# sharinka0715/semantic-gaussians

Measured on NVIDIA H100. Metric: Mviews/s + HBM GB/s, 1M Gaussians, 256-ch features, 1080p, fwd+bwd, higher is better.
Workload: dtype f32

## Files before the change

### semantic-gaussians_b200/csrc/blend_bwd.cu

```cuda
#include <cstdlib>
#include "common.cuh"

namespace sgb {

namespace {

constexpr int kThreads = SGB_TILE_PIX;
constexpr int kWarps = kThreads / 32;
constexpr int kBatchB = 32;
constexpr int CH = 4;

struct __align__(16) BwdSmem {
    float4 recA[2][kBatchB];
    float4 recB[2][kBatchB];
    uint32_t ids[2][kBatchB];
    float feat[2][kBatchB][CH];
    float dF[kWarps][kBatchB][CH];
    float geo[kWarps][kBatchB][8];
    uint32_t active[kWarps];
};

__device__ __forceinline__ float warp_sum(float v) {
#pragma unroll
    for (int o = 16; o >= 1; o >>= 1) v += __shfl_xor_sync(0xffffffffu, v, o);
    return v;
}

__global__ void __launch_bounds__(kThreads) blend_backward_kernel(
    const uint2* __restrict__ ranges, const uint32_t* __restrict__ point_list, int W, int H, int C,
    const float* __restrict__ bg_color, const SplatRec* __restrict__ rec, const float* __restrict__ colors,
    const float* __restrict__ final_Ts, const uint32_t* __restrict__ n_contrib,
    const uint32_t* __restrict__ tile_last, const float* __restrict__ dL_dpixels, float* __restrict__ dL_dmean2D,
    float* __restrict__ dL_dconic2D, float* __restrict__ dL_dopacity, float* __restrict__ dL_dcolors) {
    extern __shared__ __align__(128) unsigned char smem_raw[];
    BwdSmem& sm = *reinterpret_cast<BwdSmem*>(smem_raw);

    const int tiles_x = (W + SGB_TILE - 1) / SGB_TILE;
    const int tile = blockIdx.x;
    const int ch0 = blockIdx.y * CH;
    const int nch = min(CH, C - ch0);
    const int tid = threadIdx.x, lane = tid & 31, warp = tid >> 5;
    const uint32_t tx = tid & (SGB_TILE - 1), ty = tid >> 4;
    const uint2 pix = {(uint32_t)(tile % tiles_x) * SGB_TILE + tx, (uint32_t)(tile / tiles_x) * SGB_TILE + ty};
    const uint32_t pix_id = W * pix.y + pix.x;
    const float2 pixf = {(float)pix.x, (float)pix.y};
    const bool inside = pix.x < (uint32_t)W && pix.y < (uint32_t)H;
    const uint2 range = ranges[tile];
    const int total = (int)min(tile_last[tile], range.y - range.x);
    const int nbatches = (total + kBatchB - 1) / kBatchB;
    if (nbatches == 0) return;

    if (nch < CH)
        for (int e = tid; e < 2 * kBatchB * CH; e += kThreads) {
            const int k = e % CH;
            if (k >= nch) (&sm.feat[0][0][0])[e] = 0.f;
        }
    __syncthreads();

    auto issue = [&](int b) {
        const int st = b & 1;
        const int hi = total - b * kBatchB;
        const int cnt = min(kBatchB, hi);
        if (tid < cnt) {
            const uint32_t id = point_list[range.x + hi - 1 - tid];
            sm.ids[st][tid] = id;
            const float4* rp = reinterpret_cast<const float4*>(rec + id);
            sm.recA[st][tid] = __ldg(rp);
            sm.recB[st][tid] = __ldg(rp + 1);
        }
        for (int e = tid; e < cnt * nch; e += kThreads) {
            const int j = e / nch, k = e - j * nch;
            const uint32_t id = point_list[range.x + hi - 1 - j];
            sm.feat[st][j][k] = __ldg(colors + (size_t)id * C + ch0 + k);
        }
    };

    float dL[CH];
    float bgdot = 0.f;
    const size_t plane = (size_t)H * W;
#pragma unroll
    for (int k = 0; k < CH; k++) {
        dL[k] = (inside && k < nch) ? __ldg(dL_dpixels + (size_t)(ch0 + k) * plane + pix_id) : 0.f;
        if (k < nch) bgdot += bg_color[ch0 + k] * dL[k];
    }
    const float T_final = inside ? final_Ts[pix_id] : 0.f;
    float T = T_final;
    const int last_contributor = inside ? (int)n_contrib[pix_id] : 0;
    float last_alpha = 0.f, s_last = 0.f, A = 0.f;
    const float ddelx_dx = 0.5f * W, ddely_dy = 0.5f * H;

    issue(0);
    for (int b = 0; b < nbatches; b++) {
        const int st = b & 1;
        const int hi = total - b * kBatchB;
        const int cnt = min(kBatchB, hi);
        __syncthreads();
        if (b + 1 < nbatches) issue(b + 1);
        __syncthreads();
        uint32_t my_active = 0;

        for (int j = 0; j < cnt; j++) {
            const int pos = hi - 1 - j;
            const float4 a = sm.recA[st][j];
            const float4 con_o = sm.recB[st][j];
            const float2 d = {a.x - pixf.x, a.y - pixf.y};
            const float power = -0.5f * (con_o.x * d.x * d.x + con_o.z * d.y * d.y) - con_o.y * d.x * d.y;
            const float G = exp(power);
            const float alpha = min(0.99f, con_o.w * G);
            const bool contributes = (pos < last_contributor) && !(power > 0.0f) && !(alpha < 1.0f / 255.0f);
            if (!__any_sync(0xffffffffu, contributes)) continue;

            float w = 0.f, g0 = 0.f, g1 = 0.f, g2 = 0.f, g3 = 0.f, g4 = 0.f, g5 = 0.f;
            if (contributes) {
                T = T / (1.f - alpha);
                w = alpha * T;
                float s = 0.f;
#pragma unroll
                for (int k = 0; k < CH; k++) s += sm.feat[st][j][k] * dL[k];
                A = last_alpha * s_last + (1.f - last_alpha) * A;
                s_last = s;
                float dL_dalpha = (s - A) * T;
                last_alpha = alpha;
                dL_dalpha += (-T_final / (1.f - alpha)) * bgdot;
                const float dL_dG = con_o.w * dL_dalpha;
                const float gdx = G * d.x, gdy = G * d.y;
                const float dG_ddelx = -gdx * con_o.x - gdy * con_o.y;
                const float dG_ddely = -gdy * con_o.z - gdx * con_o.y;
                g0 = dL_dG * dG_ddelx * ddelx_dx;
                g1 = dL_dG * dG_ddely * ddely_dy;
                g2 = -0.5f * gdx * d.x * dL_dG;
                g3 = -0.5f * gdx * d.y * dL_dG;
                g4 = -0.5f * gdy * d.y * dL_dG;
                g5 = G * dL_dalpha;
            }
            g0 = warp_sum(g0); g1 = warp_sum(g1); g2 = warp_sum(g2);
            g3 = warp_sum(g3); g4 = warp_sum(g4); g5 = warp_sum(g5);
            if (lane == 0) {
                float* gp = sm.geo[warp][j];
                *reinterpret_cast<float4*>(gp) = make_float4(g0, g1, g2, g3);
                *reinterpret_cast<float2*>(gp + 4) = make_float2(g4, g5);
            }
#pragma unroll
            for (int k = 0; k < CH; k++) {
                const float t = warp_sum(w * dL[k]);
                if (lane == 0) sm.dF[warp][j][k] = t;
            }
            my_active |= 1u << j;
        }
        if (lane == 0) sm.active[warp] = my_active;
        __syncthreads();

        for (int e = tid; e < cnt * CH; e += kThreads) {
            const int j = e / CH, k = e - j * CH;
            if (k >= nch) continue;
            float t = 0.f;
            bool any = false;
#pragma unroll
            for (int wv = 0; wv < kWarps; wv++)
                if (sm.active[wv] >> j & 1u) { t += sm.dF[wv][j][k]; any = true; }
            if (any) red_add_f32(dL_dcolors + (size_t)sm.ids[st][j] * C + ch0 + k, t);
        }
        for (int e = tid; e < cnt * 6; e += kThreads) {
            const int j = e / 6, q = e - j * 6;
            float t = 0.f;
            bool any = false;
#pragma unroll
            for (int wv = 0; wv < kWarps; wv++)
                if (sm.active[wv] >> j & 1u) { t += sm.geo[wv][j][q]; any = true; }
            if (any) {
                const size_t id = sm.ids[st][j];
                float* dst = q < 2 ? dL_dmean2D + id * 3 + q
                           : q < 5 ? dL_dconic2D + id * 4 + (q == 4 ? 3 : q - 2)
                                   : dL_dopacity + id;
                red_add_f32(dst, t);
            }
        }
    }
}

}

int launch_blend_backward(const sgb_view_inputs& in, GeomView g, BinView b, ImgView im, const float* colors,
                          const float* dL_dpix, float* dL_dmean2D, float* dL_dconic, float* dL_dopacity,
                          float* dL_dcolors, cudaStream_t s) {
    if (in.C > 4) {
        set_error("launch_blend_backward handles C <= 4 only");
        return SGB_E_INVALID;
    }
    const int tiles = ((in.W + SGB_TILE - 1) / SGB_TILE) * ((in.H + SGB_TILE - 1) / SGB_TILE);
    const int chunks = (in.C + CH - 1) / CH;
    const size_t smem = sizeof(BwdSmem);
    static DeviceOnce attr_set;
    if (attr_set.first_use_on_device()) {
        SGB_CUDA(cudaFuncSetAttribute(blend_backward_kernel, cudaFuncAttributeMaxDynamicSharedMemorySize, (int)smem));
    }
    blend_backward_kernel<<<dim3(tiles, chunks), kThreads, smem, s>>>(
        im.ranges, b.point_list, in.W, in.H, in.C, in.background, g.rec, colors, im.final_T, im.n_contrib,
        im.tile_last, dL_dpix, dL_dmean2D, dL_dconic, dL_dopacity, dL_dcolors);
    SGB_LAUNCH_CHECK("blend_backward_kernel", in.debug, s);
    return SGB_OK;
}

}
```

### semantic-gaussians_b200/csrc/blend_fwd.cu

```cuda
#include <cstdlib>
#include "common.cuh"

namespace sgb {

namespace {

constexpr int kThreads = SGB_TILE_PIX;
constexpr int kBatch = 64;
constexpr int CH = 4;

struct __align__(16) FwdStage {
    float4 recA[kBatch];
    float4 recB[kBatch];
    float feat[kBatch][CH];
};

template <bool DEPTH>
__global__ void __launch_bounds__(kThreads) blend_forward_kernel(
    const uint2* __restrict__ ranges, const uint32_t* __restrict__ point_list, int W, int H, int C,
    const SplatRec* __restrict__ rec, const float* __restrict__ features, const float* __restrict__ bg_color,
    float* __restrict__ final_T, uint32_t* __restrict__ n_contrib, uint32_t* __restrict__ tile_last,
    float* __restrict__ out_color, float* __restrict__ out_depth) {
    extern __shared__ __align__(128) unsigned char smem_raw[];
    FwdStage* stage = reinterpret_cast<FwdStage*>(smem_raw);
    __shared__ uint32_t s_last;

    const int tiles_x = (W + SGB_TILE - 1) / SGB_TILE;
    const int tile = blockIdx.x;
    const int ch0 = blockIdx.y * CH;
    const int nch = min(CH, C - ch0);
    const int tid = threadIdx.x;
    const uint32_t tx = tid & (SGB_TILE - 1), ty = tid >> 4;
    const uint2 pix_min = {(uint32_t)(tile % tiles_x) * SGB_TILE, (uint32_t)(tile / tiles_x) * SGB_TILE};
    const uint2 pix = {pix_min.x + tx, pix_min.y + ty};
    const uint32_t pix_id = W * pix.y + pix.x;
    const float2 pixf = {(float)pix.x, (float)pix.y};
    const bool inside = pix.x < (uint32_t)W && pix.y < (uint32_t)H;
    bool done = !inside;

    const uint2 range = ranges[tile];
    const int total = (int)(range.y - range.x);
    const int nbatches = (total + kBatch - 1) / kBatch;

    if (tid == 0) s_last = 0;
    __syncthreads();

    auto issue = [&](int b) {
        FwdStage& st = stage[b & 1];
        const int base = b * kBatch;
        const int cnt = min(kBatch, total - base);
        if (tid < cnt) {
            const uint32_t id = point_list[range.x + base + tid];
            const float4* rp = reinterpret_cast<const float4*>(rec + id);
            st.recA[tid] = __ldg(rp);
            st.recB[tid] = __ldg(rp + 1);
        }
        for (int e = tid; e < cnt * nch; e += kThreads) {
            const int j = e / nch, k = e - j * nch;
            const uint32_t id = point_list[range.x + base + j];
            st.feat[j][k] = __ldg(features + (size_t)id * C + ch0 + k);
        }
    };

    float T = 1.0f;
    uint32_t contributor = 0;
    uint32_t last_contributor = 0;
    float D = 15.0f;
    float acc[CH];
#pragma unroll
    for (int k = 0; k < CH; k++) acc[k] = 0.f;

    if (nbatches > 0) issue(0);

    for (int b = 0; b < nbatches; b++) {
        const int num_done = __syncthreads_count(done);
        if (num_done == kThreads) break;
        if (b + 1 < nbatches) issue(b + 1);
        __syncthreads();

        const FwdStage& st = stage[b & 1];
        const int cnt = min(kBatch, total - b * kBatch);
        for (int j = 0; !done && j < cnt; j++) {
            contributor++;
            const float4 a = st.recA[j];
            const float2 xy = {a.x, a.y};
            const float2 d = {xy.x - pixf.x, xy.y - pixf.y};
            const float4 con_o = st.recB[j];
            const float power = -0.5f * (con_o.x * d.x * d.x + con_o.z * d.y * d.y) - con_o.y * d.x * d.y;
            if (power > 0.0f) continue;
            const float alpha = min(0.99f, con_o.w * exp(power));
            if (alpha < 1.0f / 255.0f) continue;
            const float test_T = T * (1 - alpha);
            if (test_T < 0.0001f) {
                done = true;
                continue;
            }
#pragma unroll
            for (int k = 0; k < CH; k++)
                if (k < nch) acc[k] += st.feat[j][k] * alpha * T;
            if (DEPTH) {
                if (T > 0.5f && test_T < 0.5) D = a.z;
            }
            T = test_T;
            last_contributor = contributor;
        }
    }

    if (blockIdx.y == 0) {
        if (inside) {
            final_T[pix_id] = T;
            n_contrib[pix_id] = last_contributor;
            if (DEPTH) out_depth[pix_id] = D;
            atomicMax(&s_last, last_contributor);
        }
        __syncthreads();
        if (tid == 0) tile_last[tile] = s_last;
    }
    if (inside) {
        const size_t plane = (size_t)H * W;
#pragma unroll
        for (int k = 0; k < CH; k++)
            if (k < nch) out_color[(size_t)(ch0 + k) * plane + pix_id] = acc[k] + T * bg_color[ch0 + k];
    }
}

template <bool DEPTH>
int launch_one(const sgb_view_inputs& in, GeomView g, BinView b, ImgView im, const float* colors,
               float* out_color, float* out_depth, cudaStream_t s) {
    const int tiles = ((in.W + SGB_TILE - 1) / SGB_TILE) * ((in.H + SGB_TILE - 1) / SGB_TILE);
    const int chunks = (in.C + CH - 1) / CH;
    const size_t smem = 2 * sizeof(FwdStage);
    auto kern = blend_forward_kernel<DEPTH>;
    static DeviceOnce attr_set;
    if (attr_set.first_use_on_device()) {
        SGB_CUDA(cudaFuncSetAttribute(kern, cudaFuncAttributeMaxDynamicSharedMemorySize, (int)smem));
    }
    kern<<<dim3(tiles, chunks), kThreads, smem, s>>>(im.ranges, b.point_list, in.W, in.H, in.C, g.rec, colors,
                                                    in.background, im.final_T, im.n_contrib, im.tile_last,
                                                    out_color, out_depth);
    SGB_LAUNCH_CHECK("blend_forward_kernel", in.debug, s);
    return SGB_OK;
}

}

int launch_blend_forward(const sgb_view_inputs& in, GeomView g, BinView b, ImgView im, const float* colors,
                         float* out_color, float* out_depth, cudaStream_t s) {
    if (in.C > 4) {
        set_error("launch_blend_forward handles C <= 4 only");
        return SGB_E_INVALID;
    }
    if (out_depth) return launch_one<true>(in, g, b, im, colors, out_color, out_depth, s);
    return launch_one<false>(in, g, b, im, colors, out_color, nullptr, s);
}

}
```

### semantic-gaussians_b200/csrc/blend_v3.cu

```cuda
#include <cstddef>
#include <cstring>
#include <cuda.h>
#include "common.cuh"
#include "blend_pool.cuh"

namespace sgb {

namespace {

constexpr int kThreads = SGB_TILE_PIX;

__device__ __forceinline__ int lane_group8(int lane) { return (lane & 1) | (((lane >> 2) & 3) << 1); }
__device__ __forceinline__ int lane_group4(int lane) { return ((lane >> 1) & 1) | ((lane >> 4) << 1); }

constexpr int kAB = 32;

struct __align__(16) AlphaSmem {
    float4 recA[kAB];
    float4 recB[kAB];
    uint32_t ids[kAB];
    float wbuf[kAB][SGB_TILE_PIX];
    uint32_t wmask[8];
    uint32_t slot_chunk[kAB];
    uint32_t cur_chunk;
    uint32_t s_last;
};

__global__ void __launch_bounds__(kThreads) alpha_pass_kernel(
    const uint2* __restrict__ ranges, const uint32_t* __restrict__ point_list, int W, int H,
    const SplatRec* __restrict__ rec, float* __restrict__ final_T, uint32_t* __restrict__ n_contrib,
    uint32_t* __restrict__ tile_last, PoolView pool) {
    extern __shared__ __align__(128) unsigned char smem_raw[];
    AlphaSmem& sm = *reinterpret_cast<AlphaSmem*>(smem_raw);

    const int tiles_x = (W + SGB_TILE - 1) / SGB_TILE;
    const int tile = blockIdx.x;
    const int tid = threadIdx.x, lane = tid & 31, warp = tid >> 5;
    const uint32_t tx = tid & (SGB_TILE - 1), ty = tid >> 4;
    const uint2 pix = {(uint32_t)(tile % tiles_x) * SGB_TILE + tx, (uint32_t)(tile / tiles_x) * SGB_TILE + ty};
    const uint32_t pix_id = W * pix.y + pix.x;
    const float2 pixf = {(float)pix.x, (float)pix.y};
    const bool inside = pix.x < (uint32_t)W && pix.y < (uint32_t)H;
    bool done = !inside;

    const uint2 range = ranges[tile];
    const int total = (int)(range.y - range.x);
    const int nbatches = (total + kAB - 1) / kAB;
    const uint32_t dbase = range.x / kChunkEntries + (uint32_t)tile;
    if (tid == 0) { sm.cur_chunk = kNone; sm.s_last = 0; }

    float T = 1.0f;
    uint32_t last_contributor = 0;
    uint32_t n_tile = 0;
    uint32_t n_blend = 0;

    auto load_id = [&](int bb) -> uint32_t {
        const int i = bb * kAB + tid;
        return (tid < kAB && bb < nbatches && i < total) ? __ldg(point_list + range.x + i) : 0u;
    };
    uint32_t id_cur = load_id(0), id_nxt = load_id(1);
    float4 rA = make_float4(0.f, 0.f, 0.f, 0.f), rB = rA;
    if (tid < kAB && tid < total) {
        const float4* rp = reinterpret_cast<const float4*>(rec + id_cur);
        rA = __ldg(rp);
        rB = __ldg(rp + 1);
    }
    for (int b = 0; b < nbatches; b++) {
        const int num_done = __syncthreads_count(done);
        if (num_done == kThreads) break;
        const int base = b * kAB;
        const int cnt = min(kAB, total - base);
        if (tid < cnt) {
            sm.ids[tid] = id_cur;
            sm.recA[tid] = rA;
            sm.recB[tid] = rB;
        }
        __syncthreads();
        if (tid < kAB) {
            id_cur = id_nxt;
            if (base + kAB + tid < total) {
                const float4* rp = reinterpret_cast<const float4*>(rec + id_cur);
                rA = __ldg(rp);
                rB = __ldg(rp + 1);
            }
            id_nxt = load_id(b + 2);
        }
        uint32_t my_mask = 0;
        for (int j = 0; j < cnt; j++) {
            float w = 0.f;
            if (!done) {
                const float4 a = sm.recA[j];
                const float2 xy = {a.x, a.y};
                const float2 d = {xy.x - pixf.x, xy.y - pixf.y};
                const float4 con_o = sm.recB[j];
                const float power = -0.5f * (con_o.x * d.x * d.x + con_o.z * d.y * d.y) - con_o.y * d.x * d.y;
                if (!(power > 0.0f)) {
                    const float alpha = min(0.99f, con_o.w * exp(power));
                    if (!(alpha < 1.0f / 255.0f)) {
                        const float test_T = T * (1 - alpha);
                        if (test_T < 0.0001f) {
                            done = true;
                        } else {
                            w = alpha * T;
                            T = test_T;
                            last_contributor = (uint32_t)(base + j + 1);
                        }
                    }
                }
            }
            sm.wbuf[j][tid] = w;
            n_blend += (w != 0.f);
            if (__ballot_sync(0xffffffffu, w != 0.f)) my_mask |= 1u << j;
        }
        if (lane == 0) sm.wmask[warp] = my_mask;
        __syncthreads();
        uint32_t tm = 0;
#pragma unroll
        for (int q = 0; q < 8; q++) tm |= sm.wmask[q];
        const int n_act = __popc(tm);
        if (n_act) {
            if (tid == 0) {
                uint32_t e = n_tile, cur = sm.cur_chunk;
                for (int k = 0; k < n_act; k++, e++) {
                    if ((e & (kChunkEntries - 1)) == 0) {
                        uint32_t nw = atomicAdd(&pool.hdr->counter, 1u);
                        if (nw >= pool.capacity) {
                            pool.hdr->overflow = 1;
                            nw = pool.capacity - 1;
                        }
                        pool.dir[dbase + e / kChunkEntries] = nw;
                        cur = nw;
                    }
                    sm.slot_chunk[k] = cur;
                }
                sm.cur_chunk = cur;
            }
            __syncthreads();
            int k = 0;
            for (uint32_t m = tm; m; m &= m - 1, k++) {
                const int j = __ffs(m) - 1;
                const uint32_t e = n_tile + k;
                WChunk& ck = pool.chunks[sm.slot_chunk[k]];
                const int s = e & (kChunkEntries - 1);
                ck.w[s][tid] = sm.wbuf[j][tid];
                if (tid == 0) {
                    uint32_t strips = 0;
#pragma unroll
                    for (int q = 0; q < 8; q++) strips |= ((sm.wmask[q] >> j) & 1u) << q;
                    ck.meta[s] = make_uint2(sm.ids[j], strips);
                }
            }
            n_tile += n_act;
        }
    }
    if (inside) {
        final_T[pix_id] = T;
        n_contrib[pix_id] = last_contributor;
        atomicMax(&sm.s_last, last_contributor);
    }
    n_blend = __reduce_add_sync(0xffffffffu, n_blend);
    if (lane == 0 && n_blend) atomicAdd(&pool.hdr->blended, (unsigned long long)n_blend);
    __syncthreads();
    if (tid == 0) {
        tile_last[tile] = sm.s_last;
        pool.count[tile] = n_tile;
        pool.dirbase[tile] = dbase;
    }
}

template <int MCH>
__device__ __forceinline__ bool acc_nonfinite(const float2 (&acc)[8][MCH / 2]) {
    float2 z = make_float2(0.f, 0.f);
#pragma unroll
    for (int i = 0; i < 8; i++)
#pragma unroll
        for (int k = 0; k < MCH / 2; k++) z = ffma2(acc[i][k], make_float2(0.f, 0.f), z);
    const float t = z.x + z.y;
    return __any_sync(0xffffffffu, t != t);
}

template <int MCH, bool RING>
__device__ __noinline__ void forward_redo_guarded(const PoolView& pool, uint32_t n, uint32_t dbase,
                                                  const float* __restrict__ features, int C, int ch0, int nch,
                                                  int warp, int woff, int cg, const float* __restrict__ bg_color,
                                                  const float* __restrict__ final_T, int W, int H, uint32_t row,
                                                  uint32_t col0, float* __restrict__ out_color) {
    float acc[8][MCH];
#pragma unroll
    for (int i = 0; i < 8; i++)
#pragma unroll
        for (int k = 0; k < MCH; k++) acc[i][k] = 0.f;
    for (uint32_t e = 0; e < n; e++) {
        const WChunk* ck = pool.chunks + chunk_of(pool, dbase, (int)(e / kChunkEntries));
        const int s = (int)(e & (kChunkEntries - 1));
        const uint2 meta = ck->meta[s];
        if (!((meta.y >> warp) & 1u)) continue;
        const float* fr = features + (size_t)meta.x * C + ch0;
        float f[MCH];
#pragma unroll
        for (int k = 0; k < MCH; k++) {
            const int chl = RING ? ((k >> 2) * 32 + cg * 4 + (k & 3)) : (cg * MCH + k);
            f[k] = chl < nch ? __ldg(fr + chl) : 0.f;
        }
#pragma unroll
        for (int i = 0; i < 8; i++) {
            const float w = ck->w[s][woff + i];
            if (w != 0.f) {
#pragma unroll
                for (int k = 0; k < MCH; k++) acc[i][k] = fmaf(f[k], w, acc[i][k]);
            }
        }
    }
    if (row >= (uint32_t)H) return;
    const size_t plane = (size_t)H * W;
#pragma unroll
    for (int k = 0; k < MCH; k++) {
        const int chl = RING ? ((k >> 2) * 32 + cg * 4 + (k & 3)) : (cg * MCH + k);
        if (chl >= nch) continue;
        const float bgc = bg_color[ch0 + chl];
        float* dst = out_color + (size_t)(ch0 + chl) * plane + (size_t)W * row + col0;
#pragma unroll
        for (int i = 0; i < 8; i++)
            if (col0 + i < (uint32_t)W) dst[i] = acc[i][k] + final_T[(size_t)W * row + col0 + i] * bgc;
    }
}

template <int CH>
__global__ void __launch_bounds__(kThreads, 2) blend_forward_v3_kernel(
    int W, int H, int C, const float* __restrict__ features, const float* __restrict__ bg_color,
    const float* __restrict__ final_T, PoolView pool, float* __restrict__ out_color) {
    constexpr int MCH = CH / 8;
    const int tiles_x = (W + SGB_TILE - 1) / SGB_TILE;
    const int nchunksC = (C + CH - 1) / CH;
    const int tile = blockIdx.x / nchunksC;
    const int ch0 = (blockIdx.x % nchunksC) * CH;
    const int nch = min(CH, C - ch0);
    const int tid = threadIdx.x, lane = tid & 31, warp = tid >> 5;
    const int pg = lane >> 3, cg = lane & 7;
    const uint2 pix_min = {(uint32_t)(tile % tiles_x) * SGB_TILE, (uint32_t)(tile / tiles_x) * SGB_TILE};

    float2 acc[8][MCH / 2];
#pragma unroll
    for (int i = 0; i < 8; i++)
#pragma unroll
        for (int k = 0; k < MCH / 2; k++) acc[i][k] = make_float2(0.f, 0.f);

    const uint32_t n = pool.count[tile];
    const uint32_t dbase = pool.dirbase[tile];
    const int woff = warp * 32 + pg * 8;
    const int foff = ch0 + cg * MCH;
    for (uint32_t e = 0; e < n;) {
        const WChunk* ck = pool.chunks + chunk_of(pool, dbase, (int)(e / kChunkEntries));
        const int m = (int)min((uint32_t)kChunkEntries, n - e);
        for (int s = 0; s < m; s++) {
            const uint2 meta = ck->meta[s];
            if (!((meta.y >> warp) & 1u)) continue;
            const float4* wp = reinterpret_cast<const float4*>(&ck->w[s][woff]);
            const float4 w0 = wp[0], w1 = wp[1];
            const float* fr = features + (size_t)meta.x * C + foff;
            float2 f[MCH / 2];
#pragma unroll
            for (int k = 0; k < MCH / 2; k++) {
                f[k].x = (cg * MCH + 2 * k < nch) ? __ldg(fr + 2 * k) : 0.f;
                f[k].y = (cg * MCH + 2 * k + 1 < nch) ? __ldg(fr + 2 * k + 1) : 0.f;
            }
            const float wv[8] = {w0.x, w0.y, w0.z, w0.w, w1.x, w1.y, w1.z, w1.w};
#pragma unroll
            for (int i = 0; i < 8; i++) {
                const float2 w2 = make_float2(wv[i], wv[i]);
#pragma unroll
                for (int k = 0; k < MCH / 2; k++) acc[i][k] = ffma2(f[k], w2, acc[i][k]);
            }
        }
        e += m;
    }
    const uint32_t row = pix_min.y + 2 * warp + (pg >> 1);
    const uint32_t col0 = pix_min.x + (pg & 1) * 8;
    if (acc_nonfinite<MCH>(acc)) {
        forward_redo_guarded<MCH, false>(pool, n, dbase, features, C, ch0, nch, warp, woff, cg, bg_color, final_T, W, H,
                                         row, col0, out_color);
        return;
    }
    if (row < (uint32_t)H) {
        const size_t plane = (size_t)H * W;
        const bool vec = ((W & 3) == 0) && (col0 + 8 <= (uint32_t)W);
        float Tv[8];
#pragma unroll
        for (int i = 0; i < 8; i++) Tv[i] = (col0 + i < (uint32_t)W) ? final_T[(size_t)W * row + col0 + i] : 0.f;
#pragma unroll
        for (int k = 0; k < MCH; k++) {
            const int chl = cg * MCH + k;
            if (chl >= nch) continue;
            const float bgc = bg_color[ch0 + chl];
            float* dst = out_color + (size_t)(ch0 + chl) * plane + (size_t)W * row + col0;
            float o[8];
#pragma unroll
            for (int i = 0; i < 8; i++) o[i] = ((k & 1) ? acc[i][k / 2].y : acc[i][k / 2].x) + Tv[i] * bgc;
            if (vec) {
                reinterpret_cast<float4*>(dst)[0] = make_float4(o[0], o[1], o[2], o[3]);
                reinterpret_cast<float4*>(dst)[1] = make_float4(o[4], o[5], o[6], o[7]);
            } else {
#pragma unroll
                for (int i = 0; i < 8; i++)
                    if (col0 + i < (uint32_t)W) dst[i] = o[i];
            }
        }
    }
}

__device__ __forceinline__ void tma_tile3d_g2s(void* dst_smem, const CUtensorMap* map, int x, int y, int z, uint64_t* bar) {
    asm volatile(
        "cp.async.bulk.tensor.3d.shared::cluster.global.tile.mbarrier::complete_tx::bytes [%0], [%1, {%2, %3, %4}], [%5];" ::"r"(
            smem_u32(dst_smem)),
        "l"(reinterpret_cast<uint64_t>(map)), "r"(x), "r"(y), "r"(z), "r"(smem_u32(bar))
        : "memory");
}
__device__ __forceinline__ void fence_proxy_async_smem() { asm volatile("fence.proxy.async.shared::cta;" ::: "memory"); }

template <int CH, int NS>
__global__ void __launch_bounds__(kThreads, 2) blend_forward_tma_kernel(
    int W, int H, int C, const float* __restrict__ features, const float* __restrict__ bg_color,
    const float* __restrict__ final_T, PoolView pool, float* __restrict__ out_color) {
    constexpr int MCH = CH / 8;
    constexpr int ES = kChunkEntries;
    constexpr int LA = NS - 2;
    constexpr int kDirCap = 192;
    struct Stage {
        float w[ES][SGB_TILE_PIX];
        float f[ES][CH];
    };
    extern __shared__ __align__(128) unsigned char smem_raw[];
    Stage* stg = reinterpret_cast<Stage*>(smem_raw);
    __shared__ uint64_t full_bar[NS], empty_bar[NS];
    __shared__ uint32_t Cdir[kDirCap];
    __shared__ __align__(16) float Tsm[SGB_TILE_PIX];
    __shared__ float bgS[CH];

    const int tiles_x = (W + SGB_TILE - 1) / SGB_TILE;
    const int nchunksC = (C + CH - 1) / CH;
    const int tile = blockIdx.x / nchunksC;
    const int ch0 = (blockIdx.x % nchunksC) * CH;
    const int nch = min(CH, C - ch0);
    const int tid = threadIdx.x, lane = tid & 31, warp = tid >> 5;
    const int pg = lane_group4(lane), cg = lane_group8(lane);
    const uint2 pix_min = {(uint32_t)(tile % tiles_x) * SGB_TILE, (uint32_t)(tile / tiles_x) * SGB_TILE};

    const uint32_t n = pool.count[tile];
    const int nb = (int)((n + ES - 1) / ES);
    const uint32_t dbase = pool.dirbase[tile];
    if (tid == 0) {
        for (int i = 0; i < NS; i++) {
            mbar_init(&full_bar[i], 1);
            mbar_init(&empty_bar[i], kThreads / 32);
        }
        mbar_fence_init();
    }
    for (int k = tid; k < min(nb, kDirCap); k += kThreads) Cdir[k] = chunk_of(pool, dbase, k);
    {
        const uint32_t x = pix_min.x + (tid & (SGB_TILE - 1)), y = pix_min.y + (tid >> 4);
        Tsm[tid] = (x < (uint32_t)W && y < (uint32_t)H) ? final_T[(size_t)W * y + x] : 0.f;
        if (tid < nch) bgS[tid] = bg_color[ch0 + tid];
    }
    if (nch < CH)
        for (int e = tid; e < NS * ES * CH; e += kThreads) {
            const int k = e % CH;
            if (k >= nch) stg[e / (ES * CH)].f[(e / CH) % ES][k] = 0.f;
        }
    __syncthreads();

    auto chunk_ptr = [&](int bi) {
        return pool.chunks + (bi < kDirCap ? Cdir[bi] : chunk_of(pool, dbase, bi));
    };
    auto load_meta = [&](int bi) {
        uint2 m = make_uint2(0u, 0u);
        if (bi < nb && lane < min(ES, (int)n - bi * ES)) m = __ldg(&chunk_ptr(bi)->meta[lane]);
        return m;
    };
    auto issue = [&](int bi, uint2 meta) {
        const int st = bi % NS;
        const int cnt = min(ES, (int)n - bi * ES);
        if (bi >= NS) mbar_wait(&empty_bar[st], (uint32_t)(((bi / NS) - 1) & 1));
        if (lane < cnt) {
            const WChunk* ck = chunk_ptr(bi);
            bulk_g2s(&stg[st].w[lane][0], &ck->w[lane][0], SGB_TILE_PIX * 4u, &full_bar[st]);
            bulk_g2s(&stg[st].f[lane][0], features + (size_t)meta.x * C + ch0, (uint32_t)nch * 4u, &full_bar[st]);
        }
        __syncwarp();
        if (lane == 0) mbar_arrive_expect_tx(&full_bar[st], (uint32_t)cnt * (SGB_TILE_PIX * 4u + (uint32_t)nch * 4u));
    };
    uint2 meta_next = make_uint2(0u, 0u);
    int pb = 0;
    if (warp == 0) {
        uint2 m[LA];
#pragma unroll
        for (int i = 0; i < LA; i++) m[i] = load_meta(i);
#pragma unroll
        for (int i = 0; i < LA; i++)
            if (i < nb) issue(i, m[i]);
        pb = min(LA, nb);
        meta_next = load_meta(pb);
    }

    float2 acc[8][MCH / 2];
#pragma unroll
    for (int i = 0; i < 8; i++)
#pragma unroll
        for (int k = 0; k < MCH / 2; k++) acc[i][k] = make_float2(0.f, 0.f);

    const int woff = warp * 32 + pg * 8;
    auto entry = [&](const Stage& sg, int e) {
        const float4 w0 = *reinterpret_cast<const float4*>(&sg.w[e][woff]);
        const float4 w1 = *reinterpret_cast<const float4*>(&sg.w[e][woff + 4]);
        float2 f[MCH / 2];
#pragma unroll
        for (int q = 0; q < MCH / 4; q++) {
            const float4 t = *reinterpret_cast<const float4*>(&sg.f[e][q * 32 + cg * 4]);
            f[2 * q] = make_float2(t.x, t.y);
            f[2 * q + 1] = make_float2(t.z, t.w);
        }
        const float wv[8] = {w0.x, w0.y, w0.z, w0.w, w1.x, w1.y, w1.z, w1.w};
#pragma unroll
        for (int i = 0; i < 8; i++) {
            const float2 w2 = make_float2(wv[i], wv[i]);
#pragma unroll
            for (int k = 0; k < MCH / 2; k++) acc[i][k] = ffma2(f[k], w2, acc[i][k]);
        }
    };
    for (int b = 0; b < nb; b++) {
        const int st = b % NS;
        const int cnt = min(ES, (int)n - b * ES);
        if (warp == 0 && pb < nb) {
            issue(pb, meta_next);
            pb++;
            meta_next = load_meta(pb);
        }
        mbar_wait(&full_bar[st], (uint32_t)((b / NS) & 1));
        if (cnt == ES) {
#pragma unroll
            for (int e = 0; e < ES; e++) entry(stg[st], e);
        } else {
            for (int e = 0; e < cnt; e++) entry(stg[st], e);
        }
        __syncwarp();
        if (lane == 0) mbar_arrive(&empty_bar[st]);
    }
    const uint32_t row = pix_min.y + 2 * warp + (pg >> 1);
    const uint32_t col0 = pix_min.x + (pg & 1) * 8;
    if (acc_nonfinite<MCH>(acc)) {
        forward_redo_guarded<MCH, true>(pool, n, dbase, features, C, ch0, nch, warp, woff, cg, bg_color, final_T, W, H,
                                        row, col0, out_color);
        return;
    }
    if (row < (uint32_t)H) {
        const size_t plane = (size_t)H * W;
        const bool vec = ((W & 3) == 0) && (col0 + 8 <= (uint32_t)W);
// ... 863 lines not shown
```

### semantic-gaussians_b200/csrc/common.cuh

```cuda
#pragma once
#include <cstdint>
#include <cstdio>
#include <cuda_runtime.h>
#include "../../include/sgb200.h"

#define SGB_TILE_PIX (SGB_TILE * SGB_TILE)

namespace sgb {

void set_error(const char* fmt, ...);
int cuda_fail(cudaError_t e, const char* what);
#define SGB_CUDA(call)                                            \
    do {                                                          \
        cudaError_t e__ = (call);                                 \
        if (e__ != cudaSuccess) return sgb::cuda_fail(e__, #call); \
    } while (0)
#define SGB_LAUNCH_CHECK(what, dbg, stream)                                   \
    do {                                                                      \
        cudaError_t e__ = cudaGetLastError();                                 \
        if (e__ == cudaSuccess && (dbg)) e__ = cudaStreamSynchronize(stream); \
        if (e__ != cudaSuccess) return sgb::cuda_fail(e__, what);             \
    } while (0)

struct __align__(16) SplatRec {
    float mx, my;
    float depth;
    float pad;
    float cx, cy, cz, op;
};
static_assert(sizeof(SplatRec) == 32, "SplatRec must be 32 bytes");

static inline size_t align_up(size_t x, size_t a = 256) { return (x + a - 1) / a * a; }

struct GeomView {
    SplatRec* rec;
    float* cov3D;
    float* rgb;
    uint8_t* clamped;
    uint32_t* tiles_touched;
    size_t bytes;
    static GeomView carve(void* base, int64_t P) {
        GeomView g;
        char* p = (char*)base;
        size_t off = 0;
        g.rec = (SplatRec*)(p + off); off += align_up(sizeof(SplatRec) * P);
        g.cov3D = (float*)(p + off); off += align_up(sizeof(float) * 6 * P);
        g.rgb = (float*)(p + off); off += align_up(sizeof(float) * 3 * P);
        g.clamped = (uint8_t*)(p + off); off += align_up(3 * (size_t)P);
        g.tiles_touched = (uint32_t*)(p + off); off += align_up(sizeof(uint32_t) * P);
        g.bytes = off;
        return g;
    }
};

struct BinView {
    uint32_t* point_list;
    size_t bytes;
    static BinView carve(void* base, int64_t R) {
        BinView b;
        b.point_list = (uint32_t*)base;
        b.bytes = align_up(sizeof(uint32_t) * (size_t)(R > 0 ? R : 1));
        return b;
    }
};

struct ImgView {
    float* final_T;
    uint32_t* n_contrib;
    uint2* ranges;
    uint32_t* tile_last;
    size_t bytes;
    static ImgView carve(void* base, int W, int H) {
        ImgView v;
        char* p = (char*)base;
        size_t N = (size_t)W * H;
        size_t tiles = (size_t)((W + SGB_TILE - 1) / SGB_TILE) * ((H + SGB_TILE - 1) / SGB_TILE);
        size_t off = 0;
        v.final_T = (float*)(p + off); off += align_up(4 * N);
        v.n_contrib = (uint32_t*)(p + off); off += align_up(4 * N);
        v.ranges = (uint2*)(p + off); off += align_up(8 * tiles);
        v.tile_last = (uint32_t*)(p + off); off += align_up(4 * tiles);
        v.bytes = off;
        return v;
    }
};

static inline sgb_view_inputs with_camera(const sgb_view_inputs& in, const sgb_camera& cam) {
    sgb_view_inputs o = in;
    o.viewmatrix = cam.viewmatrix;
    o.projmatrix = cam.projmatrix;
    o.campos = cam.campos;
    o.tan_fovx = cam.tan_fovx;
    o.tan_fovy = cam.tan_fovy;
    return o;
}

struct ViewState {
    sgb_view_inputs in;
    int64_t R;
    GeomView g;
    BinView b;
    ImgView im;
    const float* colors;
    static ViewState carve(const sgb_view_inputs& shared, const sgb_camera& cam, int64_t num_rendered,
                           const void* geometry_state, const void* binning_state, const void* image_state) {
        ViewState w;
        w.in = with_camera(shared, cam);
        w.R = w.in.P > 0 ? num_rendered : 0;
        w.g = GeomView::carve(const_cast<void*>(geometry_state), w.in.P > 0 ? w.in.P : 1);
        w.b = BinView::carve(const_cast<void*>(binning_state), w.R);
        w.im = ImgView::carve(const_cast<void*>(image_state), w.in.W, w.in.H);
        w.colors = w.in.colors_precomp ? w.in.colors_precomp : w.g.rgb;
        return w;
    }
};

struct Scratch {
    void* p = nullptr;
    size_t cap = 0;
    int ensure(size_t n);
};

}

namespace sgb {
enum Stage {
    ST_PREPROCESS = 0, ST_DEPTH_SORT, ST_SCAN, ST_EMIT, ST_TILE_SORT, ST_RANGES, ST_BLEND_FWD,
    ST_BLEND_BWD, ST_GEOM_BWD, ST_FUSION_PROJECT, ST_FUSION_SORT, ST_FUSION_GATHER, ST_ALPHA, ST_DFEATURE,
    ST_COUNT
};
constexpr int kProfRing = 320;
struct Profiler {
    bool on = false;
    cudaEvent_t ev[ST_COUNT][kProfRing][2];
    int n[ST_COUNT];
    bool created = false;
};
}

namespace sgb {
constexpr int kNumSMs = 132;

struct PoolSlot {
    Scratch mem;
    bool valid = false;
    const void* key_bin = nullptr;
    int64_t key_R = 0;
    int key_W = 0, key_H = 0, key_P = 0;
    uint32_t chunks = 0;
    uint64_t stamp = 0;
};
}

struct sgb_ctx {
    int device = 0;
    sgb::Profiler prof;
    uint64_t launches = 0;
    uint64_t lib_launches = 0;
    sgb::Scratch geom;
    sgb::Scratch bin;
    sgb::Scratch misc;
    sgb::Scratch work;
    sgb::PoolSlot pools[SGB_MAX_BATCH];
    uint64_t pool_clock = 0;
    uint64_t pool_chunks_hint = 0;
    int64_t* pinned = nullptr;
    int64_t stat_blended_pairs = 0;
    int64_t stat_pool_chunks = 0;
    cudaEvent_t feature_grad_event = nullptr;
    int64_t last_P = 0;
    int last_V = 0;
    uint32_t* d_perm[SGB_MAX_BATCH] = {};
    uint32_t* d_offsets[SGB_MAX_BATCH] = {};
};

namespace sgb {

struct StageTimer {
    sgb_ctx* c; int st; cudaStream_t s; int slot;
    StageTimer(sgb_ctx* ctx, int stage, cudaStream_t stream) : c(ctx), st(stage), s(stream), slot(-1) {
        if (c && c->prof.on && c->prof.n[st] < kProfRing) {
            slot = c->prof.n[st]++;
            cudaEventRecord(c->prof.ev[st][slot][0], s);
        }
    }
    ~StageTimer() {
        if (slot >= 0) cudaEventRecord(c->prof.ev[st][slot][1], s);
    }
};

struct DeviceOnce {
    bool done[64] = {};
    bool first_use_on_device() {
        int dev = 0;
        cudaGetDevice(&dev);
        if (dev < 0 || dev >= 64) return true;
        if (done[dev]) return false;
        done[dev] = true;
        return true;
    }
};

int launch_preprocess(const sgb_view_inputs& in, GeomView g, int32_t* radii, uint32_t* depth_keys,
                      cudaStream_t s);
int launch_mark_visible(int P, const float* means3D, const float* view, uint8_t* present, cudaStream_t s);
int run_depth_order_and_scan(sgb_ctx* ctx, const sgb_view_inputs& in, int V, const sgb_camera* cams,
                             void* const* geometry_states, int32_t* const* radii, int64_t* R_host, cudaStream_t s);
int reserve_binning(sgb_ctx* ctx, const sgb_view_inputs& in, int64_t R, cudaStream_t s);
int run_binning(sgb_ctx* ctx, const sgb_view_inputs& in, int view_slot, int64_t R, GeomView g, BinView b, ImgView im,
                const int32_t* radii, cudaStream_t s);
int launch_blend_forward(const sgb_view_inputs& in, GeomView g, BinView b, ImgView im, const float* colors,
                         float* out_color, float* out_depth, cudaStream_t s);
int launch_blend_backward(const sgb_view_inputs& in, GeomView g, BinView b, ImgView im, const float* colors,
                          const float* dL_dpix, float* dL_dmean2D, float* dL_dconic, float* dL_dopacity,
                          float* dL_dcolors, cudaStream_t s);
struct PoolView;
int weight_pool_build(sgb_ctx* ctx, const ViewState& w, cudaStream_t s);
int weight_pool_settle(sgb_ctx* ctx, int V, const ViewState* vw, PoolView* pv, cudaStream_t s,
                       const bool* only = nullptr);
int weight_rows_for_backward(sgb_ctx* ctx, int V, const ViewState* vw, PoolView* pv, cudaStream_t s);
int blend_forward_v3(sgb_ctx* ctx, const ViewState& w, const PoolView& pv, float* out_color, cudaStream_t s);
int blend_backward_v3_dfeature(sgb_ctx* ctx, const ViewState& w, const PoolView& pv, const float* dL_dpix,
                               float* dL_dcolors, cudaStream_t s);
int blend_backward_v3_chain(sgb_ctx* ctx, const ViewState& w, const PoolView& pv, const float* dL_dpix,
                            float* dL_dmean2D, float* dL_dconic, float* dL_dopacity, cudaStream_t s);
int launch_geom_backward(const sgb_view_inputs& in, GeomView g, const int32_t* radii, const float* cov3D,
                         const float* dL_dcolor_rgb, const sgb_view_grads& gr, cudaStream_t s);

#ifdef __CUDACC__
__device__ __forceinline__ uint32_t smem_u32(const void* p) {
    return (uint32_t)__cvta_generic_to_shared(p);
}
__device__ __forceinline__ void mbar_init(uint64_t* bar, uint32_t count) {
    asm volatile("mbarrier.init.shared::cta.b64 [%0], %1;" ::"r"(smem_u32(bar)), "r"(count) : "memory");
}
__device__ __forceinline__ void mbar_fence_init() {
    asm volatile("fence.mbarrier_init.release.cluster;" ::: "memory");
}
__device__ __forceinline__ void mbar_arrive_expect_tx(uint64_t* bar, uint32_t bytes) {
    asm volatile("mbarrier.arrive.expect_tx.shared::cta.b64 _, [%0], %1;" ::"r"(smem_u32(bar)), "r"(bytes)
                 : "memory");
}
__device__ __forceinline__ void mbar_arrive(uint64_t* bar) {
    asm volatile("mbarrier.arrive.shared::cta.b64 _, [%0];" ::"r"(smem_u32(bar)) : "memory");
}
__device__ __forceinline__ void mbar_wait(uint64_t* bar, uint32_t parity) {
    uint32_t done = 0;
    for (uint32_t spins = 0; !done; spins++) {
        asm volatile(
            "{\n\t.reg .pred p;\n\t"
            "mbarrier.try_wait.parity.shared::cta.b64 p, [%1], %2;\n\t"
            "selp.u32 %0, 1, 0, p;\n\t}"
            : "=r"(done)
            : "r"(smem_u32(bar)), "r"(parity)
            : "memory");
        if (spins > (1u << 24)) __trap();
    }
}
__device__ __forceinline__ void bulk_g2s(void* dst_smem, const void* src_gmem, uint32_t bytes, uint64_t* bar) {
    asm volatile("cp.async.bulk.shared::cluster.global.mbarrier::complete_tx::bytes [%0], [%1], %2, [%3];" ::"r"(
                     smem_u32(dst_smem)),
                 "l"(src_gmem), "r"(bytes), "r"(smem_u32(bar))
                 : "memory");
}
__device__ __forceinline__ float2 ffma2(float2 a, float2 b, float2 c) {
    return make_float2(fmaf(a.x, b.x, c.x), fmaf(a.y, b.y, c.y));
}
__device__ __forceinline__ void get_rect(const float2 p, int max_radius, uint2& rect_min, uint2& rect_max,
                                         dim3 grid) {
    rect_min = {min(grid.x, max((int)0, (int)((p.x - max_radius) / SGB_TILE))),
                min(grid.y, max((int)0, (int)((p.y - max_radius) / SGB_TILE)))};
    rect_max = {min(grid.x, max((int)0, (int)((p.x + max_radius + SGB_TILE - 1) / SGB_TILE))),
                min(grid.y, max((int)0, (int)((p.y + max_radius + SGB_TILE - 1) / SGB_TILE)))};
}
__device__ __forceinline__ float4 ldg_nc_f4(const float* p) {
    return __ldg(reinterpret_cast<const float4*>(p));
}
__device__ __forceinline__ void red_add_f32(float* addr, float v) {
    asm volatile("red.global.add.f32 [%0], %1;" ::"l"(addr), "f"(v) : "memory");
}
__device__ __forceinline__ void red_add_v4_f32(float* addr, float4 v) {
    asm volatile("red.global.add.v4.f32 [%0], {%1, %2, %3, %4};" ::"l"(addr), "f"(v.x), "f"(v.y), "f"(v.z),
                 "f"(v.w)
                 : "memory");
}
#endif

}
```

Before: 0.00005090.

## Cull splats that cannot reach a tile before blending in all blend kernels

Measured after the change: 0.00005228 (median of 6 runs). 1.03x the previous value.

```diff
diff --git a/semantic-gaussians_b200/csrc/blend_bwd.cu b/semantic-gaussians_b200/csrc/blend_bwd.cu
--- a/semantic-gaussians_b200/csrc/blend_bwd.cu
+++ b/semantic-gaussians_b200/csrc/blend_bwd.cu
@@ -18,6 +18,7 @@
     float dF[kWarps][kBatchB][CH];
     float geo[kWarps][kBatchB][8];
     uint32_t active[kWarps];
+    uint32_t live[2];
 };
 
 __device__ __forceinline__ float warp_sum(float v) {
@@ -61,12 +62,19 @@
         const int st = b & 1;
         const int hi = total - b * kBatchB;
         const int cnt = min(kBatchB, hi);
-        if (tid < cnt) {
-            const uint32_t id = point_list[range.x + hi - 1 - tid];
-            sm.ids[st][tid] = id;
-            const float4* rp = reinterpret_cast<const float4*>(rec + id);
-            sm.recA[st][tid] = __ldg(rp);
-            sm.recB[st][tid] = __ldg(rp + 1);
+        if (tid < kBatchB) {
+            bool live = false;
+            if (tid < cnt) {
+                const uint32_t id = point_list[range.x + hi - 1 - tid];
+                sm.ids[st][tid] = id;
+                const float4* rp = reinterpret_cast<const float4*>(rec + id);
+                const float4 ra = __ldg(rp), rb = __ldg(rp + 1);
+                sm.recA[st][tid] = ra;
+                sm.recB[st][tid] = rb;
+                live = !splat_cannot_reach_tile(ra, rb, tile, tiles_x, W, H);
+            }
+            const uint32_t m = __ballot_sync(0xffffffffu, live);
+            if (tid == 0) sm.live[st] = m;
         }
         for (int e = tid; e < cnt * nch; e += kThreads) {
             const int j = e / nch, k = e - j * nch;
@@ -99,7 +107,8 @@
         __syncthreads();
         uint32_t my_active = 0;
 
-        for (int j = 0; j < cnt; j++) {
+        for (uint32_t lm = sm.live[st]; lm; lm &= lm - 1) {
+            const int j = __ffs(lm) - 1;
             const int pos = hi - 1 - j;
             const float4 a = sm.recA[st][j];
             const float4 con_o = sm.recB[st][j];
diff --git a/semantic-gaussians_b200/csrc/blend_fwd.cu b/semantic-gaussians_b200/csrc/blend_fwd.cu
--- a/semantic-gaussians_b200/csrc/blend_fwd.cu
+++ b/semantic-gaussians_b200/csrc/blend_fwd.cu
@@ -8,11 +8,13 @@
 constexpr int kThreads = SGB_TILE_PIX;
 constexpr int kBatch = 64;
 constexpr int CH = 4;
+static_assert(kBatch == 64, "the live mask of a stage is one 64-bit word");
 
 struct __align__(16) FwdStage {
     float4 recA[kBatch];
     float4 recB[kBatch];
     float feat[kBatch][CH];
+    uint32_t live[kBatch / 32];
 };
 
 template <bool DEPTH>
@@ -49,11 +51,18 @@
         FwdStage& st = stage[b & 1];
         const int base = b * kBatch;
         const int cnt = min(kBatch, total - base);
-        if (tid < cnt) {
-            const uint32_t id = point_list[range.x + base + tid];
-            const float4* rp = reinterpret_cast<const float4*>(rec + id);
-            st.recA[tid] = __ldg(rp);
-            st.recB[tid] = __ldg(rp + 1);
+        if (tid < kBatch) {
+            bool live = false;
+            if (tid < cnt) {
+                const uint32_t id = point_list[range.x + base + tid];
+                const float4* rp = reinterpret_cast<const float4*>(rec + id);
+                const float4 ra = __ldg(rp), rb = __ldg(rp + 1);
+                st.recA[tid] = ra;
+                st.recB[tid] = rb;
+                live = !splat_cannot_reach_tile(ra, rb, tile, tiles_x, W, H);
+            }
+            const uint32_t m = __ballot_sync(0xffffffffu, live);
+            if ((tid & 31) == 0) st.live[tid >> 5] = m;
         }
         for (int e = tid; e < cnt * nch; e += kThreads) {
             const int j = e / nch, k = e - j * nch;
@@ -79,9 +88,9 @@
         __syncthreads();
 
         const FwdStage& st = stage[b & 1];
-        const int cnt = min(kBatch, total - b * kBatch);
-        for (int j = 0; !done && j < cnt; j++) {
-            contributor++;
+        for (uint64_t lm = st.live[0] | (uint64_t)st.live[1] << 32; !done && lm; lm &= lm - 1) {
+            const int j = __ffsll((long long)lm) - 1;
+            contributor = (uint32_t)(b * kBatch + j + 1);
             const float4 a = st.recA[j];
             const float2 xy = {a.x, a.y};
             const float2 d = {xy.x - pixf.x, xy.y - pixf.y};
diff --git a/semantic-gaussians_b200/csrc/blend_v3.cu b/semantic-gaussians_b200/csrc/blend_v3.cu
--- a/semantic-gaussians_b200/csrc/blend_v3.cu
+++ b/semantic-gaussians_b200/csrc/blend_v3.cu
@@ -22,6 +22,9 @@
     float wbuf[kAB][SGB_TILE_PIX];
     uint32_t wmask[8];
     uint32_t slot_chunk[kAB];
+    uint32_t seg_id[kThreads];
+    uint32_t seg_pos[kThreads];
+    uint32_t seg_mask[8];
     uint32_t cur_chunk;
     uint32_t s_last;
 };
@@ -45,7 +48,6 @@
 
     const uint2 range = ranges[tile];
     const int total = (int)(range.y - range.x);
-    const int nbatches = (total + kAB - 1) / kAB;
     const uint32_t dbase = range.x / kChunkEntries + (uint32_t)tile;
     if (tid == 0) { sm.cur_chunk = kNone; sm.s_last = 0; }
 
@@ -54,103 +56,122 @@
     uint32_t n_tile = 0;
     uint32_t n_blend = 0;
 
-    auto load_id = [&](int bb) -> uint32_t {
-        const int i = bb * kAB + tid;
-        return (tid < kAB && bb < nbatches && i < total) ? __ldg(point_list + range.x + i) : 0u;
-    };
-    uint32_t id_cur = load_id(0), id_nxt = load_id(1);
-    float4 rA = make_float4(0.f, 0.f, 0.f, 0.f), rB = rA;
-    if (tid < kAB && tid < total) {
-        const float4* rp = reinterpret_cast<const float4*>(rec + id_cur);
-        rA = __ldg(rp);
-        rB = __ldg(rp + 1);
-    }
-    for (int b = 0; b < nbatches; b++) {
-        const int num_done = __syncthreads_count(done);
-        if (num_done == kThreads) break;
-        const int base = b * kAB;
-        const int cnt = min(kAB, total - base);
-        if (tid < cnt) {
-            sm.ids[tid] = id_cur;
-            sm.recA[tid] = rA;
-            sm.recB[tid] = rB;
-        }
+    for (int seg = 0; seg < total; seg += kThreads) {
+        if (__syncthreads_count(done) == kThreads) break;
+        const int i = seg + tid;
+        uint32_t id = 0;
+        bool live = false;
+        if (i < total) {
+            id = __ldg(point_list + range.x + i);
+            const float4* rp = reinterpret_cast<const float4*>(rec + id);
+            live = !splat_cannot_reach_tile(__ldg(rp), __ldg(rp + 1), tile, tiles_x, W, H);
+        }
+        const uint32_t bal = __ballot_sync(0xffffffffu, live);
+        if (lane == 0) sm.seg_mask[warp] = bal;
         __syncthreads();
-        if (tid < kAB) {
-            id_cur = id_nxt;
-            if (base + kAB + tid < total) {
+        int n_live = 0, rank = 0;
+#pragma unroll
+        for (int q = 0; q < 8; q++) {
+            const int c = __popc(sm.seg_mask[q]);
+            rank += q < warp ? c : 0;
+            n_live += c;
+        }
+        if (live) {
+            rank += __popc(bal & ((1u << lane) - 1u));
+            sm.seg_id[rank] = id;
+            sm.seg_pos[rank] = (uint32_t)i;
+        }
+        __syncthreads();
+
+        uint32_t id_cur = 0;
+        float4 rA = make_float4(0.f, 0.f, 0.f, 0.f), rB = rA;
+        auto load_round = [&](int k) {
+            if (tid < kAB && k + tid < n_live) {
+                id_cur = sm.seg_id[k + tid];
                 const float4* rp = reinterpret_cast<const float4*>(rec + id_cur);
                 rA = __ldg(rp);
                 rB = __ldg(rp + 1);
             }
-            id_nxt = load_id(b + 2);
-        }
-        uint32_t my_mask = 0;
-        for (int j = 0; j < cnt; j++) {
-            float w = 0.f;
-            if (!done) {
-                const float4 a = sm.recA[j];
-                const float2 xy = {a.x, a.y};
-                const float2 d = {xy.x - pixf.x, xy.y - pixf.y};
-                const float4 con_o = sm.recB[j];
-                const float power = -0.5f * (con_o.x * d.x * d.x + con_o.z * d.y * d.y) - con_o.y * d.x * d.y;
-                if (!(power > 0.0f)) {
-                    const float alpha = min(0.99f, con_o.w * exp(power));
-                    if (!(alpha < 1.0f / 255.0f)) {
-                        const float test_T = T * (1 - alpha);
-                        if (test_T < 0.0001f) {
-                            done = true;
-                        } else {
-                            w = alpha * T;
-                            T = test_T;
-                            last_contributor = (uint32_t)(base + j + 1);
+        };
+        load_round(0);
+        for (int k = 0; k < n_live; k += kAB) {
+            if (k > 0 && __syncthreads_count(done) == kThreads) break;
+            const int cnt = min(kAB, n_live - k);
+            if (tid < cnt) {
+                sm.ids[tid] = id_cur;
+                sm.recA[tid] = rA;
+                sm.recB[tid] = rB;
+            }
+            __syncthreads();
+            load_round(k + kAB);
+            uint32_t my_mask = 0;
+            const bool warp_done = __all_sync(0xffffffffu, done);
+            for (int j = 0; !warp_done && j < cnt; j++) {
+                float w = 0.f;
+                if (!done) {
+                    const float4 a = sm.recA[j];
+                    const float2 xy = {a.x, a.y};
+                    const float2 d = {xy.x - pixf.x, xy.y - pixf.y};
+                    const float4 con_o = sm.recB[j];
+                    const float power = -0.5f * (con_o.x * d.x * d.x + con_o.z * d.y * d.y) - con_o.y * d.x * d.y;
+                    if (!(power > 0.0f)) {
+                        const float alpha = min(0.99f, con_o.w * exp(power));
+                        if (!(alpha < 1.0f / 255.0f)) {
+                            const float test_T = T * (1 - alpha);
+                            if (test_T < 0.0001f) {
+                                done = true;
+                            } else {
+                                w = alpha * T;
+                                T = test_T;
+                                last_contributor = sm.seg_pos[k + j] + 1;
+                            }
                         }
                     }
                 }
-            }
-            sm.wbuf[j][tid] = w;
-            n_blend += (w != 0.f);
-            if (__ballot_sync(0xffffffffu, w != 0.f)) my_mask |= 1u << j;
-        }
-        if (lane == 0) sm.wmask[warp] = my_mask;
-        __syncthreads();
-        uint32_t tm = 0;
-#pragma unroll
-        for (int q = 0; q < 8; q++) tm |= sm.wmask[q];
-        const int n_act = __popc(tm);
-        if (n_act) {
-            if (tid == 0) {
-                uint32_t e = n_tile, cur = sm.cur_chunk;
-                for (int k = 0; k < n_act; k++, e++) {
-                    if ((e & (kChunkEntries - 1)) == 0) {
-                        uint32_t nw = atomicAdd(&pool.hdr->counter, 1u);
-                        if (nw >= pool.capacity) {
-                            pool.hdr->overflow = 1;
-                            nw = pool.capacity - 1;
+                sm.wbuf[j][tid] = w;
+                n_blend += (w != 0.f);
+                if (__ballot_sync(0xffffffffu, w != 0.f)) my_mask |= 1u << j;
+            }
+            if (lane == 0) sm.wmask[warp] = my_mask;
+            __syncthreads();
+            uint32_t tm = 0;
+#pragma unroll
+            for (int q = 0; q < 8; q++) tm |= sm.wmask[q];
+            const int n_act = __popc(tm);
+            if (n_act) {
+                if (tid == 0) {
+                    uint32_t e = n_tile, cur = sm.cur_chunk;
+                    for (int r = 0; r < n_act; r++, e++) {
+                        if ((e & (kChunkEntries - 1)) == 0) {
+                            uint32_t nw = atomicAdd(&pool.hdr->counter, 1u);
+                            if (nw >= pool.capacity) {
+                                pool.hdr->overflow = 1;
+                                nw = pool.capacity - 1;
+                            }
+                            pool.dir[dbase + e / kChunkEntries] = nw;
+                            cur = nw;
                         }
-                        pool.dir[dbase + e / kChunkEntries] = nw;
-                        cur = nw;
+                        sm.slot_chunk[r] = cur;
                     }
-                    sm.slot_chunk[k] = cur;
+                    sm.cur_chunk = cur;
                 }
-                sm.cur_chunk = cur;
-            }
-            __syncthreads();
-            int k = 0;
-            for (uint32_t m = tm; m; m &= m - 1, k++) {
-                const int j = __ffs(m) - 1;
-                const uint32_t e = n_tile + k;
-                WChunk& ck = pool.chunks[sm.slot_chunk[k]];
-                const int s = e & (kChunkEntries - 1);
-                ck.w[s][tid] = sm.wbuf[j][tid];
-                if (tid == 0) {
-                    uint32_t strips = 0;
-#pragma unroll
-                    for (int q = 0; q < 8; q++) strips |= ((sm.wmask[q] >> j) & 1u) << q;
-                    ck.meta[s] = make_uint2(sm.ids[j], strips);
+                __syncthreads();
+                int r = 0;
+                for (uint32_t m = tm; m; m &= m - 1, r++) {
+                    const int j = __ffs(m) - 1;
+                    const uint32_t e = n_tile + r;
+                    WChunk& ck = pool.chunks[sm.slot_chunk[r]];
+                    const int s = e & (kChunkEntries - 1);
+                    ck.w[s][tid] = warp_done ? 0.f : sm.wbuf[j][tid];
+                    if (tid == 0) {
+                        uint32_t strips = 0;
+#pragma unroll
+                        for (int q = 0; q < 8; q++) strips |= ((sm.wmask[q] >> j) & 1u) << q;
+                        ck.meta[s] = make_uint2(sm.ids[j], strips);
+                    }
                 }
-            }
-            n_tile += n_act;
+                n_tile += n_act;
+            }
         }
     }
     if (inside) {
diff --git a/semantic-gaussians_b200/csrc/common.cuh b/semantic-gaussians_b200/csrc/common.cuh
--- a/semantic-gaussians_b200/csrc/common.cuh
+++ b/semantic-gaussians_b200/csrc/common.cuh
@@ -1,4 +1,5 @@
 #pragma once
+#include <cmath>
 #include <cstdint>
 #include <cstdio>
 #include <cuda_runtime.h>
@@ -227,6 +228,42 @@
 int launch_geom_backward(const sgb_view_inputs& in, GeomView g, const int32_t* radii, const float* cov3D,
                          const float* dL_dcolor_rgb, const sgb_view_grads& gr, cudaStream_t s);
 
+#if defined(__CUDACC__)
+#define SGB_HD __host__ __device__ __forceinline__
+#else
+#define SGB_HD inline
+#endif
+
+SGB_HD bool splat_cannot_reach(float mx, float my, float a, float b, float c, float op, float x0, float y0, float x1,
+                               float y1) {
+    const float dx0 = mx - x1, dx1 = mx - x0, dy0 = my - y1, dy1 = my - y0;
+    const float lim_d = 1e9f, lim_k = 1e18f;
+    if (!(fabsf(dx0) <= lim_d && fabsf(dx1) <= lim_d && fabsf(dy0) <= lim_d && fabsf(dy1) <= lim_d)) return false;
+    if (!(a >= 1e-18f && c >= 1e-18f && a <= lim_k && c <= lim_k && fabsf(b) <= lim_k && fabsf(op) <= lim_k))
+        return false;
+    const float ac = a * c;
+    const float den = fmaf(a, c, -b * b) - 1e-6f * ac;
+    if (!(den > 0.f)) return false;
+    float q = 0.f;
+    if (!(dx0 <= 0.f && dx1 >= 0.f && dy0 <= 0.f && dy1 >= 0.f)) {
+#if defined(__CUDA_ARCH__)
+        const float b_c = __fdividef(b, c), b_a = __fdividef(b, a);
+#else
+        const float b_c = b / c, b_a = b / a;
+#endif
+        const float tx0 = fminf(fmaxf(-b_c * dx0, dy0), dy1), tx1 = fminf(fmaxf(-b_c * dx1, dy0), dy1);
+        const float ty0 = fminf(fmaxf(-b_a * dy0, dx0), dx1), ty1 = fminf(fmaxf(-b_a * dy1, dx0), dx1);
+        const float q0 = (a * dx0 + 2.f * b * tx0) * dx0 + c * tx0 * tx0;
+        const float q1 = (a * dx1 + 2.f * b * tx1) * dx1 + c * tx1 * tx1;
+        const float q2 = (c * dy0 + 2.f * b * ty0) * dy0 + a * ty0 * ty0;
+        const float q3 = (c * dy1 + 2.f * b * ty1) * dy1 + a * ty1 * ty1;
+        q = fminf(fminf(q0, q1), fminf(q2, q3));
+    }
+    const float u = 5.9604645e-8f;
+    const float L = logf(255.f * op);
+    return 0.5f * q * fmaxf(0.f, den - 1.5263e-5f * ac) > (L + 64.f * u * (1.f + fabsf(L))) * den;
+}
+
 #ifdef __CUDACC__
 __device__ __forceinline__ uint32_t smem_u32(const void* p) {
     return (uint32_t)__cvta_generic_to_shared(p);
@@ -273,6 +310,11 @@
     rect_max = {min(grid.x, max((int)0, (int)((p.x + max_radius + SGB_TILE - 1) / SGB_TILE))),
                 min(grid.y, max((int)0, (int)((p.y + max_radius + SGB_TILE - 1) / SGB_TILE)))};
 }
+__device__ __forceinline__ bool splat_cannot_reach_tile(float4 recA, float4 recB, int tile, int tiles_x, int W, int H) {
+    const int x0 = (tile % tiles_x) * SGB_TILE, y0 = (tile / tiles_x) * SGB_TILE;
+    return splat_cannot_reach(recA.x, recA.y, recB.x, recB.y, recB.z, recB.w, (float)x0, (float)y0,
+                              (float)min(x0 + SGB_TILE - 1, W - 1), (float)min(y0 + SGB_TILE - 1, H - 1));
+}
 __device__ __forceinline__ float4 ldg_nc_f4(const float* p) {
     return __ldg(reinterpret_cast<const float4*>(p));
 }
```
